# ayankele/dune-transformercvn

Measured on AMD Instinct MI355X. Metric: events/sec (fwd+bwd) at batch=32, 8 prongs/event; fraction of MFMA roofline, higher is better.
Workload: dtype bf16; 1 GPU; TransformerCVN DenseNet [3,6,12,6,3] g32, fwd+loss+bwd, batch 32/GPU, 8 prongs/event, 3x400x280 maps, 6-layer encoder, dropout 0.1; global_batch=32, parallelism=dp1, precision=bf16

## Files before the change

dune-transformercvn_amd/csrc/conv3x3_tile.hip:

```cpp
#include <cstdlib>
#include <type_traits>
#include "tile3x3.h"
#include "prof.h"

namespace tcvn {

using namespace t3;

namespace {


__device__ __forceinline__ int fdiv(int a, int d, float inv, int& rem) {
    int q = (int)((float)a * inv);
    rem = a - q * d;
    if (rem < 0) { --q; rem += d; }
    else if (rem >= d) { ++q; rem -= d; }
    return q;
}
__device__ __forceinline__ int pix_of(const PadGeom& q, int g, float invWp, float invHp) {
    if (g < 0 || g >= (int)q.gtot) return -1;
    int wp, hp;
    const int row = fdiv(g, q.Wp, invWp, wp);
    const int img = fdiv(row, q.Hp, invHp, hp);
    if (hp < 1 || hp > q.H || wp < 1 || wp > q.W) return -1;
// ... 294 lines not shown
    const int nrows4 = (q.rows() + 3) & ~3;
    int* tbl = reinterpret_cast<int*>(smem + ring * 256);
    float* xchg = reinterpret_cast<float*>(smem + ring * 256 + PAIR_TBL * 4);
    bf16* ctile = reinterpret_cast<bf16*>(xchg + 2 * 4 * 16 * 64);
    double* red = reinterpret_cast<double*>(ctile + 4 * 32 * 32);
    float* xtab = reinterpret_cast<float*>(red + 4 * 32 * 2);

    const int tid = threadIdx.x, lane = tid & 63, wave = tid >> 6;
    const bool roleB = wave >= 4;
    const bool xf = g.act_fused != 0;
    const int pw = wave & 3;
    const int r = lane & 31, h = lane >> 5;
    const float invWp = 1.0f / q.Wp, invHp = 1.0f / q.Hp;
    const bf16* __restrict__ YA = reinterpret_cast<const bf16*>(g.Aact);
    const char* __restrict__ zeros = reinterpret_cast<const char*>(g.zeros);
    bf16* __restrict__ Out = reinterpret_cast<bf16*>(g.Out);
    const int nb = gridDim.x, base = ntiles / nb, rem = ntiles % nb;
    const int t0 = blockIdx.x * base + min((int)blockIdx.x, rem), t1 = t0 + base + ((int)blockIdx.x < rem ? 1 : 0);
    const int g_org = t0 * TP - q.halo;
    const bool nok = r < g.N;
    const float bias = nok ? g.bias[r] : 0.f;
    const bool drop = g.drop_p > 0.f;
    const uint32_t dkey = drop_key(g.seed, g.stream_id);
    const bool vec_store = g.N == 32 && (g.n_off & 7) == 0 && (g.ldo & 7) == 0 && (reinterpret_cast<uintptr_t>(g.Out) & 15) == 0;
    auto wrap = [&](int x) { return x >= ring ? x - ring : x; };

    const bf16* __restrict__ Wf = reinterpret_cast<const bf16*>(g.Wfrag) + lane * 8;

    auto fill_rows = [&](int row0, int n, int t, int nt) {
        for (int i = t; i < n; i += nt) tbl[(row0 + i) & (PAIR_TBL - 1)] = pix_of(q, g_org + row0 + i, invWp, invHp);
    };
    auto dma_rows = [&](int row0, int slot0, int n, int w0, int nw) {
        const int rsub = lane >> 4, slot = lane & 15;
        for (int rg0 = w0; rg0 * 4 < n; rg0 += 4 * nw) {
            int m4[4];
#pragma unroll
            for (int j = 0; j < 4; ++j) m4[j] = tbl[(row0 + (rg0 + nw * j) * 4 + rsub) & (PAIR_TBL - 1)];
#pragma unroll
            for (int j = 0; j < 4; ++j) {
                const int rg = rg0 + nw * j;
                if (rg * 4 < n) {
                    const int ring_row = wrap(slot0 + rg * 4);
                    const int rr = ring_row + rsub;
                    const char* src = m4[j] >= 0 ? reinterpret_cast<const char*>(YA + (long)m4[j] * 128) + ((slot ^ (rr & 15)) << 4) : zeros + (slot << 4);
                    __builtin_amdgcn_global_load_lds((const __attribute__((address_space(1))) void*)src,
                                                     (__attribute__((address_space(3))) void*)(smem + ring_row * 256), 16, 0, 0);
// ... 20 lines not shown
            const Act8 tb = act8_load(xtab, cc);
#pragma unroll
            for (int j = 0; j < 4; ++j)
                if (m4[j] >= 0) *reinterpret_cast<u16x8*>(p[j]) = act8_apply(v[j], tb);
        }
    };
    if (t0 < t1) fill_rows(0, nrows4, tid, 512);
    if (t0 + 1 < t1) fill_rows(nrows4, TP, tid, 512);
    if (xf && g.lf.isum != nullptr) {
        if (tid < 128) {
            float tsc, tsh;
            lf_table(g.lf, tid, blockIdx.x == 0, tsc, tsh);
            xtab[tid] = tsc; xtab[128 + tid] = tsh; xtab[256 + tid] = g.sl[tid];
        }
    } else if (xf) act_tab_fill(xtab, g.sc, g.sh, g.sl, tid, 512);
    __syncthreads();
    if (t0 < t1) dma_rows(0, 0, nrows4, wave, 8);

#ifdef TCVN_DEBUG_KNOBS
    unsigned long long ph[16] = {0, 0, 0, 0, 0, 0, 0, 0, 0, 0, 0, 0, 0, 0, 0, 0};
#endif
    double s1 = 0, s2 = 0;
    f32x16 accp;
#pragma unroll
    for (int e = 0; e < 16; ++e) accp[e] = 0.f;
    int slot_tile = 0;
    int slot_new = wrap(nrows4);
    auto epilogue_impl = [&](auto dropc, auto vecc, int te, const f32x16& mine) {
        constexpr bool DROP = decltype(dropc)::value, VEC = decltype(vecc)::value;
        const float* xc = xchg + (((te - t0) & 1) * 4 + pw) * 16 * 64 + lane;
        float part[16];
#pragma unroll
        for (int e = 0; e < 16; ++e) part[e] = xc[e * 64];
        int mrow[16];
#pragma unroll
        for (int e = 0; e < 16; ++e) mrow[e] = tbl[((te - t0) * TP + q.halo + pw * 32 + (e & 3) + 8 * (e >> 2) + 4 * h) & (PAIR_TBL - 1)];
        float f1 = 0.f, f2 = 0.f;
        bf16* ct = ctile + pw * 32 * 32;
        uint32_t kword = 0;
#pragma unroll
        for (int e = 0; e < 16; ++e) {
            const int m = mrow[e];
            const bool ok = m >= 0 && nok;
            float v = mine[e] + part[e] + bias;
            if (DROP) {
                const int mm = m < 0 ? 0 : m;
                const float dsc = drop_pick(drop_bits32(dkey, mm, r, g.N), mm, g.drop_p);
                v *= dsc;
                const unsigned long long bal = __ballot(dsc != 0.f);
                kword = lane == 2 * e ? (uint32_t)bal : lane == 2 * e + 1 ? (uint32_t)(bal >> 32) : kword;
            }
            const bf16 o = ok ? f2bf(v) : (bf16)0;
            const float x = bf2f(o);
            f1 += x; f2 = fmaf(x, x, f2);
            if (VEC) ct[((e & 3) + 8 * (e >> 2) + 4 * h) * 32 + r] = o;
            else if (ok) Out[(long)m * g.ldo + g.n_off + r] = o;
        }
        s1 += (double)f1; s2 += (double)f2;
        if (DROP && g.keep_out != nullptr && lane < 32) {
            const int el = lane >> 1, pos = (el & 3) + 8 * (el >> 2) + 4 * (lane & 1);
            const int m = tbl[((te - t0) * TP + q.halo + pw * 32 + pos) & (PAIR_TBL - 1)];
            if (m >= 0) g.keep_out[m] = kword;
        }
        if (VEC) {
#pragma unroll
            for (int i = 0; i < 2; ++i) {
                const int c = lane + 64 * i, pos = c >> 2, chunk = c & 3;
                const int m = tbl[((te - t0) * TP + q.halo + pw * 32 + pos) & (PAIR_TBL - 1)];
                const u16x8 v8 = *reinterpret_cast<const u16x8*>(ct + pos * 32 + chunk * 8);
                if (m >= 0) *reinterpret_cast<u16x8*>(Out + (long)m * g.ldo + g.n_off + chunk * 8) = v8;
            }
        }
    };
    auto epilogue = [&](int te, const f32x16& mine) {
        if (drop) {
            if (vec_store) epilogue_impl(std::true_type{}, std::true_type{}, te, mine);
            else epilogue_impl(std::true_type{}, std::false_type{}, te, mine);
        } else {
            if (vec_store) epilogue_impl(std::false_type{}, std::true_type{}, te, mine);
            else epilogue_impl(std::false_type{}, std::false_type{}, te, mine);
        }
    };

    auto multiply = [&](auto& bwr, auto ntc, int tap_first, int slot_t, f32x16& acc) {
        constexpr int NT = decltype(ntc)::value, NG = NT * 2;
#pragma unroll
        for (int e = 0; e < 16; ++e) acc[e] = 0.f;
        const int lrow0 = slot_t + pw * 32 + r + q.halo;
        auto row_of = [&](int tp) {
            const int tap = tap_first + tp;
            int lr = lrow0 + (tap / 3 - 1) * q.Wp + (tap % 3 - 1);
            lr = lr >= ring ? lr - ring : lr;
            return lr >= ring ? lr - ring : lr;
        };
        bf16x8_t af[2][4];
        auto load_group = [&](int gI, bf16x8_t (&dst)[4]) {
            const int lr = row_of(gI >> 1), ks0 = (gI & 1) * 4;
#pragma unroll
            for (int i = 0; i < 4; ++i)
                dst[i] = *reinterpret_cast<const bf16x8_t*>(smem + lr * 256 + (((2 * (ks0 + i) + h) ^ (lr & 15)) << 4));
        };
        load_group(0, af[0]);
#pragma unroll
// ... 34 lines not shown
            if (t + 2 < t1) fill_rows(nrows4 + (t - t0 + 1) * TP, TP, tid, 256);
            PAIR_PH(4);
            slot_tile = wrap(slot_tile + TP);
            slot_new = wrap(slot_new + TP);
        }
    } else {
        bf16x8_t bw[32];
#pragma unroll
        for (int i = 0; i < 32; ++i) bw[i] = *reinterpret_cast<const bf16x8_t*>(Wf + (40 + i) * 512);
        __builtin_amdgcn_s_setprio(1);
        PAIR_T0();
        int slot_dma = 0;
        for (int t = t0; t < t1; ++t) {
            asm volatile("s_waitcnt vmcnt(0)" ::: "memory");
            if (xf) {
                if (t == t0) xform_rows(0, 0, nrows4, wave, 8);
                else xform_rows(nrows4 + (t - 1 - t0) * TP, slot_dma, TP, wave, 8);
            }
            PAIR_PH(8);
            __syncthreads();
            PAIR_PH(9);
            slot_dma = slot_new;
            if (xf && t + 1 < t1) dma_rows(nrows4 + (t - t0) * TP, slot_new, TP, wave, 8);
            PAIR_PH(10);
            if (t > t0) epilogue(t - 1, accp);
            PAIR_PH(11);
            multiply(bw, std::integral_constant<int, 4>{}, 5, slot_tile, accp);
            PAIR_PH(12);
            slot_tile = wrap(slot_tile + TP);
            slot_new = wrap(slot_new + TP);
        }
    }
#ifdef TCVN_DEBUG_KNOBS
    if (lane == 0 && (blockIdx.x & 15) == 0)
        for (int i = 0; i < 16; ++i)
            if (ph[i]) atomicAdd(&g_pair_ph[i], ph[i]);
#endif
    __syncthreads();
    if (roleB && t1 > t0) epilogue(t1 - 1, accp);
    if (g.part != nullptr || g.isum_out != nullptr) {
        double a = s1, b = s2;
        a += __shfl_xor(a, 32); b += __shfl_xor(b, 32);
        if (roleB && lane < 32) { red[(pw * 32 + lane) * 2] = a; red[(pw * 32 + lane) * 2 + 1] = b; }
        __syncthreads();
        if (tid < g.N) {
            double x = 0, y = 0;
#pragma unroll
            for (int w = 0; w < 4; ++w) { x += red[(w * 32 + tid) * 2]; y += red[(w * 32 + tid) * 2 + 1]; }
            if (g.isum_out != nullptr) lf_add(g.isum_out, g.isum_stride, tid, x, y);
            else {
                g.part[((long)blockIdx.x * g.N + tid) * 2] = x;
                g.part[((long)blockIdx.x * g.N + tid) * 2 + 1] = y;
            }
        }
    }
}
int fwd_pair_ring(const PadGeom& q) { return (int)((((q.rows() + 3) & ~3) + TP + 15) & ~15); }
size_t fwd_pair_smem(const PadGeom& q) { const size_t ring = fwd_pair_ring(q); return ring * 256 + PAIR_TBL * 4 + 2 * 4 * 16 * 64 * 4 + 4 * 32 * 32 * 2 + 4 * 32 * 16 + 3 * 128 * 4; }


size_t fwd_smem(const PadGeom& q) { const size_t r4 = (q.rows() + 3) & ~3; return 2 * r4 * 256 + 3 * r4 * 4 + 4 * 32 * 16; }

// ... 948 lines not shown
    return q.gtot < (1L << 24) && fwd_smem(q) <= 160 * 1024;
}
int conv3x3_tile_nblk(const ConvFwdArgs& a) {
    const PadGeom q(a.M / (a.H * a.W), a.H, a.W);
    return tile_grid(q.tiles());
}
static bool fwd_strip_forced() {
    static const bool on = TCVN_KNOB_SET("TCVN_FWD_STRIP");
    return on;
}
static bool fwd_pair_ok(const ConvFwdArgs& a, const PadGeom& q) {
    return fwd_pair_smem(q) <= 160 * 1024 && 4 * TP + q.halo + q.Wp + 1 < PAIR_TBL && (long)a.M * a.N < (1L << 32) && !fwd_strip_forced();
}
bool conv3x3_act_fusable(const ConvFwdArgs& a) {
    if (!conv3x3_tile_ok(a) || a.sc == nullptr || a.sh == nullptr || a.sl == nullptr) return false;
    static const bool off = TCVN_KNOB_SET("TCVN_NO_ACT_FUSE");
    const PadGeom q(a.M / (a.H * a.W), a.H, a.W);
    return !off && fwd_pair_ok(a, q) && wgrad_smem(q) <= 160 * 1024;
}
bool conv3x3_fwd_pair(const ConvFwdArgs& a) {
    if (!conv3x3_tile_ok(a)) return false;
    return fwd_pair_ok(a, PadGeom(a.M / (a.H * a.W), a.H, a.W));
}
bool conv3x3_fwd_writes_keep(const ConvFwdArgs& a) {
    if (a.keep_out == nullptr || a.drop_p <= 0.f || !conv3x3_tile_ok(a)) return false;
    return fwd_pair_ok(a, PadGeom(a.M / (a.H * a.W), a.H, a.W));
}
int conv3x3_fwd_tile(const ConvFwdArgs& a, hipStream_t st) {
    const int n_img = a.M / (a.H * a.W);
    const PadGeom q(n_img, a.H, a.W);
    const int ntiles = (int)q.tiles();
    const int nb = tile_grid(ntiles);
    const size_t smem = fwd_smem(q);
    static bool attr = false;
    if (!attr) {
        TCVN_CHECK(hipFuncSetAttribute(reinterpret_cast<const void*>(k_conv3x3_fwd_bf16), hipFuncAttributeMaxDynamicSharedMemorySize,
                                       160 * 1024));
        attr = true;
    }
    ProfScope ps("k_conv3x3_fwd_bf16", 2.0 * a.M * (double)a.N * a.K, (double)a.M * 2.0 * (a.C + a.N), st);
    if (fwd_pair_ok(a, q)) {
        static bool attr3 = false;
        if (!attr3) {
            TCVN_CHECK(hipFuncSetAttribute(reinterpret_cast<const void*>(k_conv3x3_fwd_pair_bf16), hipFuncAttributeMaxDynamicSharedMemorySize,
                                           160 * 1024));
            attr3 = true;
        }
        hipLaunchKernelGGL(k_conv3x3_fwd_pair_bf16, dim3(nb), dim3(512), fwd_pair_smem(q), st, a, n_img, ntiles, fwd_pair_ring(q));
        TCVN_LAUNCH_CHECK();
        return 0;
// ... 124 lines not shown
```

dune-transformercvn_amd/csrc/densenet.hip:

```cpp
#include <string>
#include <vector>
#include <cstring>

#include "../../include/tcvn_hip.h"
#include "tcvn_ops.h"
#include "tcvn_rows.h"
#include <cstdlib>
#include "densenet_plan.h"

using namespace tcvn;

namespace {
constexpr float kEps = 1e-5f, kMom = 0.1f;
}

int DenseNetPlan::add_slot(const std::string& name, long numel, int kind) {
    slots.push_back({name, numel, kind});
    return (int)slots.size() - 1;
}
BnSlots DenseNetPlan::add_bn(const std::string& p, int c) {
    BnSlots s;
    s.w = add_slot(p + ".weight", c, TCVN_SLOT_PARAM);
    s.b = add_slot(p + ".bias", c, TCVN_SLOT_PARAM);
    s.rm = add_slot(p + ".running_mean", c, TCVN_SLOT_BUFFER);
// ... 239 lines not shown
}

int DenseNetPlan::bind(void* const* d, void* const* g) {
    for (size_t i = 0; i < slots.size(); ++i) {
        data[i] = reinterpret_cast<float*>(d[i]);
        grad[i] = g ? reinterpret_cast<float*>(g[i]) : nullptr;
        if (slots[i].kind != TCVN_SLOT_COUNTER && data[i] == nullptr) {
            fprintf(stderr, "tcvn: slot %s unbound\n", slots[i].name.c_str());
            return -10;
        }
    }
    wk_cache = wk_list();
    fast3x3 = cfg.mode == MODE_BF16 && cfg.bn_size * cfg.growth == 128 && cfg.growth <= 32 && conv3x3_tile_enabled();
    bound = true;
    desc_ws = nullptr;
    undesc_ws = nullptr;
    return 0;
}

namespace {
struct Tab { float* sc; float* sh; };
}

int DenseNetPlan::upload_descs(char* ws, const Layout& L, hipStream_t st) {
    if (desc_ws == ws && desc_total == L.total) return 0;
    std::vector<PackDesc> pd;
    for (const auto& e : wk_cache) {
        PackDesc d;
        d.src = data[e.slot]; d.dst = ws + L.wk + e.off; d.N = e.N; d.Cin = e.Cin; d.taps = e.taps; d.Kp = e.Kp;
        d.transpose = e.transpose; d.frag = e.frag;
        pd.push_back(d);
    }
    std::vector<BnEvalDesc> bd;
    float* tabs = reinterpret_cast<float*>(ws + L.tabs);
    auto addbn = [&](const BnSlots& s) {
        BnEvalDesc d;
        d.gamma = data[s.w]; d.beta = data[s.b]; d.rm = data[s.rm]; d.rv = data[s.rv];
        d.sc = tabs + tab_off(s); d.sh = d.sc + round_up(s.C, 8); d.C = s.C;
        bd.push_back(d);
    };
    addbn(n0);
    for (const auto& bg : blocks) {
        for (const auto& ls : bg.layers) { addbn(ls.n1); addbn(ls.n2); }
        if (bg.has_trans) addbn(bg.tn);
    }
    addbn(nf);
    n_pack = (int)pd.size(); n_bneval = (int)bd.size();
    const size_t bytes = pd.size() * sizeof(PackDesc) + bd.size() * sizeof(BnEvalDesc);
    if (bytes > desc_cap) {
        if (d_desc) TCVN_CHECK(hipFree(d_desc));
        TCVN_CHECK(hipMalloc(&d_desc, bytes));
        desc_cap = bytes;
    }
    h_desc.resize(bytes);
    memcpy(h_desc.data(), pd.data(), pd.size() * sizeof(PackDesc));
    memcpy(h_desc.data() + pd.size() * sizeof(PackDesc), bd.data(), bd.size() * sizeof(BnEvalDesc));
    TCVN_CHECK(hipMemcpyAsync(d_desc, h_desc.data(), bytes, hipMemcpyHostToDevice, st));
    desc_ws = ws; desc_total = L.total;
    return 0;
}

int DenseNetPlan::forward(int n, const int32_t* coords, const float* values, long nnz, int log_pixels, float noise_std,
                          float* out, long out_ld, char* ws, long ws_bytes, int train, uint64_t seed, hipStream_t st) {
    if (!bound) return -11;
    if (n <= 0) return 0;
    Layout L;
    layout(n, train != 0, L);
    if (ws_bytes < L.total) { fprintf(stderr, "tcvn: densenet workspace too small (%ld < %ld)\n", ws_bytes, L.total); return -12; }
    int rc;
    if ((rc = upload_descs(ws, L, st))) return rc;
    const int mode = cfg.mode, g = cfg.growth, mid = cfg.bn_size * cfg.growth;
    float* tabs = reinterpret_cast<float*>(ws + L.tabs);
    auto tab = [&](const BnSlots& s) { Tab t; t.sc = tabs + tab_off(s); t.sh = t.sc + round_up(s.C, 8); return t; };
    double* part = reinterpret_cast<double*>(ws + L.part);
    const PackDesc* d_pack = reinterpret_cast<const PackDesc*>(d_desc);
    const BnEvalDesc* d_bn = reinterpret_cast<const BnEvalDesc*>(d_desc + n_pack * sizeof(PackDesc));

    if ((rc = pack_weights(d_pack, n_pack, mode, st))) return rc;
    if (!train && (rc = bn_eval_tables(d_bn, n_bneval, kEps, st))) return rc;

    auto link = [&](const BnSlots& s, const double* prt, int nblk, int part_ld, int c_new0, int n_new, double* bstat,
                    long count, const long long* isum = nullptr, long isum_stride = 0) -> int {
        if (!train) return 0;
        BnLinkArgs a{};
        a.isum = isum; a.isum_stride = isum_stride;
        a.part = prt; a.nblk = nblk; a.part_ld = part_ld; a.c_new0 = c_new0; a.n_new = n_new; a.bstat = bstat;
        a.count = count; a.C = s.C; a.gamma = data[s.w]; a.beta = data[s.b];
        a.running_mean = data[s.rm]; a.running_var = data[s.rv];
        Tab t = tab(s); a.sc = t.sc; a.sh = t.sh; a.train = 1; a.eps = kEps; a.momentum = kMom;
        return bn_link(a, st);
    };

    static const bool no_lf = TCVN_KNOB_SET("TCVN_NO_LF");
    const bool lf_on = train && !no_lf && mode == MODE_BF16 && L.isum_bytes > 0;
    TCVN_CHECK(hipMemsetAsync(ws + L.zeros, 0, 1024 + (lf_on ? L.isum_bytes : 0), st));
    auto lf_of = [&](const BnSlots& s, const long long* isum, long rep_stride, int c_new0, int n_new, double* bstat, long count) {
        LfLink k{};
        k.isum = isum; k.rep_stride = rep_stride; k.c_new0 = c_new0; k.n_new = n_new; k.bstat = bstat; k.inv_count = 1.0 / (double)count; k.count = count;
        k.gamma = data[s.w]; k.beta = data[s.b]; k.running_mean = data[s.rm]; k.running_var = data[s.rv];
        Tab t = tab(s); k.sc_out = t.sc; k.sh_out = t.sh; k.eps = kEps; k.momentum = kMom;
        return k;
    };
// ... 170 lines not shown
                if ((int)act_fused[bi].size() != bg.L) act_fused[bi].assign(bg.L, 0);
                act_fused[bi][l] = 0;
                if (mode == MODE_BF16) {
                    a.zeros = ws + L.zeros;
                    a.Aact = ws + L.Y[bi][l];
                    if (!fuse_ya && conv3x3_act_fusable(a)) { a.act_fused = 1; act_fused[bi][l] = 1; }
                    else {
                        if (!fuse_ya) {
                            ActArgs act{ws + L.Y[bi][l], mid, M, mid, t.sc, t.sh, data[ls.a2], ws + L.YA[bi][l], mid};
                            if ((rc = act_bf16(act, st))) return rc;
                        }
                        a.Aact = ws + L.YA[bi][l];
                    }
                }
                a.part = train ? part : nullptr;
                a.drop_p = train ? cfg.dropout : 0.f; a.seed = seed; a.stream_id = (uint32_t)(bi * 64 + l + 1);
                a.nblk = conv_fwd_nblk(a);
                if (lf2) {
                    if (!a.act_fused) { fprintf(stderr, "tcvn: link-free norm2 without the in-LDS activation\n"); return -17; }
                    a.lf = lf_of(ls.n2, reinterpret_cast<long long*>(ws + L.isumY[bi][l]), 2L * mid, 0, mid, reinterpret_cast<double*>(ws + L.bstatY[bi][l]), M);
                }
                const bool out_isum = lf_on && mode == MODE_BF16 && conv3x3_fwd_pair(a) && g <= 32;
                if (out_isum) { a.isum_out = isumD + 2 * ls.cin; a.isum_stride = 2L * bg.ld; }
                if (train && !L.KM[bi].empty()) {
                    a.keep_out = reinterpret_cast<uint32_t*>(ws + L.KM[bi][l]);
                    if (keep_valid.size() != blocks.size()) keep_valid.assign(blocks.size(), std::vector<char>());
                    if ((int)keep_valid[bi].size() != bg.L) keep_valid[bi].assign(bg.L, 0);
                    keep_valid[bi][l] = conv3x3_fwd_writes_keep(a) ? 1 : 0;
                }
                if ((rc = conv_fwd(a, st))) return rc;
                new_c0 = ls.cin; new_n = g; new_nblk = a.nblk; new_ld = g; new_isum = out_isum;
            }
        }
        if (bg.has_trans) {
            const BlockGeom& nb = blocks[bi + 1];
            if ((rc = link(bg.tn, part, new_nblk, new_ld, new_c0, new_n, bstatD, M, new_isum ? isumD + 2 * new_c0 : nullptr, 2L * bg.ld))) return rc;
            const WkEntry& e = wk_find(bg.tw, 0);
            Tab t = tab(bg.tn);
            const long Mn = (long)n * nb.H * nb.W;
            const bool fastt = L.XP[bi] >= 0 && mode == MODE_BF16;
            const bool mat32 = L.XP[bi] >= 0 && mode == MODE_F32;
            if (fastt || mat32) {
                ActPoolArgs ap{D, bg.ld, n, bg.H, bg.W, bg.Ctot, t.sc, t.sh, data[bg.ta], ws + L.XP[bi], bg.ldp};
                if ((rc = fastt ? act_pool_bf16(ap, st) : act_pool_f32(ap, st))) return rc;
            }
            if (fastt) {
                const WkEntry& ef = wk_find(bg.tw, 0, 1);
                GemmNtArgs ga{};
                ga.epi = EPI_FWD; ga.A = ws + L.XP[bi]; ga.lda = bg.ldp; ga.K = bg.ldp; ga.M = Mn; ga.N = bg.Ctot / 2;
                ga.Wfrag = ws + L.wk + ef.off; ga.Kp = ef.Kp; ga.zeros = ws + L.zeros; ga.bias = data[bg.tb];
                ga.Out = ws + L.D[bi + 1]; ga.ldo = nb.ld; ga.n_off = 0; ga.part = train ? part : nullptr; ga.nblk = gemm_nt_nblk(ga);
// ... 24 lines not shown
    if ((rc = linear_fwd(F, Cf, data[s_wl], nullptr, Z, cfg.out_dim, n, cfg.out_dim, Cf, st))) return rc;
    float* hs = reinterpret_cast<float*>(ws + L.head_stat);
    RowsBnArgs r{};
    r.X = Z; r.ldx = cfg.out_dim; r.R = n; r.C = cfg.out_dim; r.gamma = data[nl.w]; r.beta = data[nl.b]; r.slope = data[s_al];
    r.running_mean = data[nl.rm]; r.running_var = data[nl.rv]; r.Y = out; r.ldy = out_ld;
    r.save_mean = hs; r.save_rstd = hs + cfg.out_dim; r.train = train; r.eps = kEps; r.momentum = kMom;
    r.drop_p = train ? cfg.dropout : 0.f; r.seed = seed; r.stream_id = 0x4000u;
    if ((rc = rows_bn_fwd(r, st))) return rc;
    last_seed = seed; last_n = n; last_coords = coords; last_nnz = nnz;
    return 0;
}

int DenseNetPlan::tap(int n, const char* name, long* off, int* tn, int* th, int* tw, int* tc, int* tld, int* tes) const {
    Layout L;
    layout(n, false, L);
    std::string s(name);
    *tn = n; *tes = esz;
    if ((s == "img" || s == "conv0") && last_sparse_stem && n == last_n) return -1;
    if (s == "img") { *off = L.img; *th = cfg.H; *tw = cfg.W; *tc = cfg.in_ch; *tld = cfg.in_ch; return 0; }
    if (s == "conv0") { *off = L.c0; *th = Hc; *tw = Wc; *tc = cfg.init_ch; *tld = cfg.init_ch; return 0; }
    if (s == "condense") { *off = L.F; *th = 1; *tw = 1; *tc = Cf; *tld = Cf; *tes = 4; return 0; }
    if (s == "raw:wk") { *tn = *th = *tw = 1; *off = L.wk; *tc = *tld = (int)(wk_bytes() / esz); return 0; }
    if (s == "raw:tabs") { *tn = *th = *tw = 1; *off = L.tabs; *tc = *tld = (int)tab_floats(); *tes = 4; return 0; }
    if (s.rfind("raw:ystat", 0) == 0) {
        int b = 0, l = 0;
        if (sscanf(s.c_str(), "raw:ystat%d.%d", &b, &l) != 2) return -1;
        b -= 1;
        if (b < 0 || b >= (int)blocks.size() || l < 0 || l >= blocks[b].L) return -1;
        *tn = *th = *tw = 1; *off = L.bstatY[b][l]; *tc = *tld = 2 * cfg.bn_size * cfg.growth; *tes = 8; return 0;
    }
    if (s.rfind("raw:bstat", 0) == 0) {
        const int b = atoi(s.c_str() + 9) - 1;
        if (b < 0 || b >= (int)blocks.size()) return -1;
        *tn = *th = *tw = 1; *off = L.bstatD[b]; *tc = *tld = blocks[b].ld * 2; *tes = 8; return 0;
    }
    if (s.rfind("dense", 0) == 0) {
        const int b = atoi(s.c_str() + 5) - 1;
        if (b < 0 || b >= (int)blocks.size()) return -1;
        *off = L.D[b]; *th = blocks[b].H; *tw = blocks[b].W; *tc = blocks[b].Ctot; *tld = blocks[b].ld;
        return 0;
    }
    if (s.rfind("bottleneck", 0) == 0) {
        int b = 0, l = 0;
        if (sscanf(s.c_str(), "bottleneck%d.%d", &b, &l) != 2) return -1;
        b -= 1;
        if (b < 0 || b >= (int)blocks.size() || l < 0 || l >= blocks[b].L) return -1;
// ... 75 lines not shown
```

dune-transformercvn_amd/csrc/densenet_plan.h:

```cpp
#pragma once
#include <string>
#include <vector>

#include "../../include/tcvn_hip.h"
#include "tcvn_common.h"

namespace tcvn {

struct Bwd1x1Args;
struct Slot { std::string name; long numel; int kind; };
struct BnSlots { int w = -1, b = -1, rm = -1, rv = -1, nbt = -1, C = 0, id = -1; };
struct LayerSlots { BnSlots n1, n2; int a1, w1, b1, a2, w2, b2, cin; };
struct BlockGeom {
    int H, W, C0, L, Ctot, ld;
    int ldp;
    std::vector<LayerSlots> layers;
    bool has_trans = false;
    BnSlots tn; int ta = -1, tw = -1, tb = -1;
};
struct WkEntry { int slot, N, Cin, taps, transpose, rows, Kp, frag; long off; };

struct Layout {
    long img, c0, bstat0, part, tabs, F, Z, head_stat, wk, fwd_end, total;
    std::vector<long> D, bstatD;
// ... 10 lines not shown
    std::vector<std::vector<long>> XA;
    std::vector<long> XP;
    long du, du0, pq0, pqY, gwk, bpart, dF, dZ, zero_end;
    std::vector<long> G, pqD;
};

bool backward_overlap_enabled();
void set_backward_overlap(int on);

struct DenseNetPlan {
    tcvn_densenet_cfg cfg;
    int esz, Hc, Wc, Cf, n_bn = 0;
    std::vector<Slot> slots;
    std::vector<float*> data, grad;
    std::vector<BlockGeom> blocks;
    int s_w0, s_b0, s_a0, s_af, s_wl, s_al;
    BnSlots n0, nf, nl;
    std::vector<WkEntry> wk_cache;
    bool bound = false;
    bool fast1_ok(int cin) const;
    bool fastt_ok(int Ctot) const;
    bool fast3x3 = false;
    char* d_desc = nullptr; size_t desc_cap = 0; std::vector<char> h_desc;
    char* desc_ws = nullptr; long desc_total = 0; int n_pack = 0, n_bneval = 0;
    uint64_t last_seed = 0; int last_n = 0;
    const int32_t* last_coords = nullptr; long last_nnz = 0;
    const float* last_values = nullptr; int last_value_mode = 0; float last_noise = 0.f;
    std::vector<std::vector<char>> keep_valid;
    std::vector<std::vector<char>> act_fused;
    std::vector<std::vector<char>> xa_skipped;
    bool last_fused_ya = false;
    bool last_stem_act = false;
    bool last_sparse_stem = false;
    bool sparse_stem_possible() const;
    hipStream_t side_st = nullptr; hipEvent_t ev_fork_a = nullptr, ev_fork_b = nullptr, ev_done[2] = {nullptr, nullptr}, ev_drain = nullptr;
    int ensure_side();
    char* d_undesc = nullptr; std::vector<char> h_undesc; char* undesc_ws = nullptr; long undesc_total = 0; int n_unpack = 0;

    explicit DenseNetPlan(const tcvn_densenet_cfg& c);
    ~DenseNetPlan();
    int add_slot(const std::string& name, long numel, int kind);
    BnSlots add_bn(const std::string& p, int c);
    void layout(int n, bool bwd, Layout& L) const;
    void layout_bwd(int n, long start, long maxY, Layout& L) const;
    long tab_floats() const;
    long tab_off(const BnSlots& s) const;
    long wk_bytes() const;
    std::vector<WkEntry> wk_list() const;
    const WkEntry& wk_find(int slot, int transpose, int frag = 0) const;
    const void* wk_frag(const char* ws, const Layout& L, int slot, int transpose) const;
    int bind(void* const* d, void* const* g);
    int upload_descs(char* ws, const Layout& L, hipStream_t st);
    int forward(int n, const int32_t* coords, const float* values, long nnz, int log_pixels, float noise_std, float* out,
                long out_ld, char* ws, long ws_bytes, int train, uint64_t seed, hipStream_t st);
    int backward(int n, const float* d_out, long d_out_ld, char* ws, long ws_bytes, hipStream_t st, int bi_hi = -1, int bi_lo = 0);
    bool bwd1x1_fill(int bi, int l, long M, char* ws, const Layout& L, Bwd1x1Args& fa) const;
    bool bwd1x1_fusable(int bi, int l, long M, char* ws, const Layout& L) const;
    std::vector<int> unpack_first;
    int tap(int n, const char* name, long* off, int* tn, int* th, int* tw, int* tc, int* tld, int* tes) const;
};

}
```

dune-transformercvn_amd/csrc/elementwise.hip:

```cpp
#include "tcvn_ops.h"

namespace tcvn {

namespace {

__global__ __launch_bounds__(256) void k_bn_link(const BnLinkArgs a) {
    const int wave = threadIdx.x >> 6, lane = threadIdx.x & 63;
    const int c = blockIdx.x * 4 + wave;
    if (c >= a.C) return;
    const float gamma = a.gamma[c], beta = a.beta[c];
    const bool upd = a.train && a.running_mean != nullptr;
    const float rmean = upd || !a.train ? a.running_mean[c] : 0.f, rvar = upd || !a.train ? a.running_var[c] : 0.f;
    double mean, var;
    if (a.train) {
        if (c >= a.c_new0 && c < a.c_new0 + a.n_new && a.isum != nullptr) {
            long long sa, sb;
            lf_sums(a.isum, a.isum_stride, c - a.c_new0, sa, sb);
            mean = (double)sa * ((1.0 / (double)a.count) / LF_S1);
            var = (double)sb * ((1.0 / (double)a.count) / LF_S2) - mean * mean;
            if (var < 0) var = 0;
            if (lane == 0) { a.bstat[c * 2] = mean; a.bstat[c * 2 + 1] = var; }
        } else if (c >= a.c_new0 && c < a.c_new0 + a.n_new) {
            double s1 = 0, s2 = 0;
            for (int b = lane; b < a.nblk; b += 512) {
// ... 285 lines not shown
        const int r = (int)(q / kc8), k0 = (int)(q - (long)r * kc8) * 8;
        float v[8];
        int tap = k0 / inner, c = k0 - tap * inner;
#pragma unroll
        for (int j = 0; j < 8; ++j) {
            v[j] = 0.f;
            if (r < rows && k0 + j < klim)
                v[j] = d.transpose ? d.src[((long)c * d.Cin + r) * d.taps + tap] : d.src[((long)r * d.Cin + c) * d.taps + tap];
            if (++c == inner) { c = 0; ++tap; }
        }
        const long o = d.frag ? ((((long)(r >> 5) * (d.Kp >> 4) + (k0 >> 4)) * 64 + ((k0 >> 3) & 1) * 32 + (r & 31)) * 8) : (long)r * d.Kp + k0;
        if constexpr (sizeof(T) == 2) {
            u16x8 w;
#pragma unroll
            for (int j = 0; j < 8; ++j) w[j] = f2bf(v[j]);
            *reinterpret_cast<u16x8*>(dst + o) = w;
        } else {
            *reinterpret_cast<f32x4*>(dst + o) = f32x4{v[0], v[1], v[2], v[3]};
            *reinterpret_cast<f32x4*>(dst + o + 4) = f32x4{v[4], v[5], v[6], v[7]};
        }
    }
}


__global__ __launch_bounds__(256) void k_pool0_vec64(const Pool0Args a) {
    __shared__ double red[4][8][8][2];
    const bf16* X = reinterpret_cast<const bf16*>(a.X);
    bf16* O = reinterpret_cast<bf16*>(a.Out);
    const int tid = threadIdx.x, c8 = tid & 7;
    float sc[8], sh[8], sl[8];
#pragma unroll
    for (int j = 0; j < 8; ++j) { sc[j] = a.sc[c8 * 8 + j]; sh[j] = a.sh[c8 * 8 + j]; sl[j] = a.sl[c8 * 8 + j]; }
    double s1[8], s2[8];
#pragma unroll
    for (int j = 0; j < 8; ++j) { s1[j] = 0; s2[j] = 0; }
    const long npix = (long)a.n_img * a.Ho * a.Wo;
    for (long p = (long)blockIdx.x * 32 + (tid >> 3); p < npix; p += (long)gridDim.x * 32) {
        const int wo = (int)(p % a.Wo);
        const int ho = (int)((p / a.Wo) % a.Ho);
        const long img = p / ((long)a.Wo * a.Ho);
        const bf16* base = X + ((img * a.Hin + 2 * ho) * a.Win + 2 * wo) * 64 + c8 * 8;
        float acc[8] = {0, 0, 0, 0, 0, 0, 0, 0};
#pragma unroll
        for (int dy = 0; dy < 3; ++dy)
#pragma unroll
            for (int dx = 0; dx < 3; ++dx) {
// ... 94 lines not shown
    hipLaunchKernelGGL(k_act_pool_bf16, dim3((unsigned)(g < 4096 ? g : 4096)), dim3(256), 3 * cpr * 8 * sizeof(float), st, a);
    TCVN_LAUNCH_CHECK();
    return 0;
}

int act_pool_f32(const ActPoolArgs& a, hipStream_t st) {
    if ((a.ldx & 3) || (a.ldo & 3) || a.ldo < a.C || (reinterpret_cast<uintptr_t>(a.X) & 15) || (reinterpret_cast<uintptr_t>(a.Out) & 15)) return -2;
    const long total = (long)a.n_img * (a.Hin / 2) * (a.Win / 2) * (a.ldo >> 2);
    if (total <= 0) return 0;
    const long g = (total + 255) / 256;
    hipLaunchKernelGGL(k_act_pool_f32, dim3((unsigned)(g < 8192 ? g : 8192)), dim3(256), 0, st, a);
    TCVN_LAUNCH_CHECK();
    return 0;
}

int pack_weights(const PackDesc* d_descs, int n, int mode, hipStream_t st) {
    if (n <= 0) return 0;
    if (mode == MODE_F32) hipLaunchKernelGGL(k_pack<float>, dim3(256, n), dim3(256), 0, st, d_descs);
    else hipLaunchKernelGGL(k_pack<bf16>, dim3(256, n), dim3(256), 0, st, d_descs);
    TCVN_LAUNCH_CHECK();
    return 0;
}

}
```

dune-transformercvn_amd/csrc/tcvn_ops.h:

```cpp
#pragma once
#include "tcvn_common.h"
#include "bn_lf.h"

namespace tcvn {

enum AMode { A_1X1 = 0, A_1X1_POOL = 1, A_3X3 = 2, A_STEM = 3 };

struct ConvFwdArgs {
    int mode, amode;
    const void* A; long lda;
    int M, N, K, Kp;
    int C, H, W, Hin, Win;
    const float *sc, *sh, *sl;
    const void* Wk; const float* bias;
    void* Out; long ldo; int n_off;
    const void* Wfrag;
    const void* Aact;
    const void* zeros;
    double* part; int nblk;
    float drop_p; uint64_t seed; uint32_t stream_id;
    uint32_t* keep_out;
    int act_fused;
    LfLink lf;
    long long* isum_out; long isum_stride;
};
int conv_fwd(const ConvFwdArgs& a, hipStream_t st);
bool conv3x3_fwd_pair(const ConvFwdArgs& a);
bool conv3x3_fwd_writes_keep(const ConvFwdArgs& a);
bool conv3x3_act_fusable(const ConvFwdArgs& a);
int conv_fwd_grid(int M);
int conv_fwd_nblk(const ConvFwdArgs& a);
bool conv3x3_tile_ok(const ConvFwdArgs& a);
int conv3x3_tile_nblk(const ConvFwdArgs& a);
int conv3x3_fwd_tile(const ConvFwdArgs& a, hipStream_t st);
bool conv3x3_tile_enabled();

struct BnLinkArgs {
    const double* part; int nblk; int part_ld;
    int c_new0, n_new;
    double* bstat;
    long count;
    int C;
    const float *gamma, *beta;
    float *running_mean, *running_var;
    float *sc, *sh;
    int train; float eps, momentum;
    const long long* isum; long isum_stride;
};
int bn_link(const BnLinkArgs& a, hipStream_t st);

struct BnEvalDesc { const float *gamma, *beta, *rm, *rv; float *sc, *sh; int C; };
int bn_eval_tables(const BnEvalDesc* d_descs, int n, float eps, hipStream_t st);

struct ScatterArgs {
    int mode; const int* coords; const float* values; long nnz; int n_img;
    void* img; int H, W, Cpix; int log_pixels; float noise_std; uint64_t seed;
};
int scatter_pixels(const ScatterArgs& a, hipStream_t st);

struct Pool0Args {
    int mode; const void* X; int n_img, Hin, Win, C; const float *sc, *sh, *sl;
    void* Out; long ldo; int Ho, Wo; double* part; int nblk;
};
int pool0_fwd(const Pool0Args& a, hipStream_t st);
int pool0_grid(int n_img, int Ho, int Wo);

struct HeadPoolArgs { int mode; const void* X; long ldx; int n_img, HW, C; const float *sc, *sh, *sl; float* F; };
int head_pool_fwd(const HeadPoolArgs& a, hipStream_t st);

struct ActArgs { const void* X; long ldx; long M; int C; const float *sc, *sh, *sl; void* Out; long ldo; };
int act_bf16(const ActArgs& a, hipStream_t st);

struct PackDesc { const float* src; void* dst; int N, Cin, taps, Kp; int transpose; int frag; };
int pack_weights(const PackDesc* d_descs, int n, int mode, hipStream_t st);

struct EffSrc {
    const void* G; long ldg;
    const void* X; long ldx;
    int c_off, N;
    const float *P, *Q;
    float drop_p; uint64_t seed; uint32_t stream_id;
    const uint32_t* keep;
    const void* ey;
};

enum DMode { DG_1X1 = 0, DG_1X1_POOL = 1, DG_3X3 = 2 };
struct ConvDgradArgs {
    int mode, dmode;
    EffSrc e;
    int M, N, Kp;
    int H, W, Hin, Win;
    const void* Wt;
    const void* Xin; long ldxin;
    const float *sc, *sh, *sl;
    void* Gout; long ldgo; int accumulate;
    double* part; int nblk;
    const void* Wfrag;
// ... 187 lines not shown
```

Baseline: 1773 events/s.

## Precompute dropout keep masks in one batched kernel, read them in conv epilogue

Adds a batched k_keep_words kernel that produces the dropout keep bitmasks for every dense layer up front. The 3x3 tile conv epilogue then loads a prefetched keep word per row and applies the mask with readlane and inverse_ballot, instead of hashing random bits per element inside the MFMA-heavy kernel. This takes RNG work off the conv critical path at the cost of one extra launch and extra mask reads and writes. Computing masks inside the kernel is still available behind an env knob.

```diff
diff --git a/dune-transformercvn_amd/csrc/conv3x3_tile.hip b/dune-transformercvn_amd/csrc/conv3x3_tile.hip
--- a/dune-transformercvn_amd/csrc/conv3x3_tile.hip
+++ b/dune-transformercvn_amd/csrc/conv3x3_tile.hip
@@ -340,6 +340,8 @@
     const float bias = nok ? g.bias[r] : 0.f;
     const bool drop = g.drop_p > 0.f;
     const uint32_t dkey = drop_key(g.seed, g.stream_id);
+    const uint32_t* __restrict__ KM = g.keep_in;
+    const float dinv = 1.f / (1.f - g.drop_p);
     const bool vec_store = g.N == 32 && (g.n_off & 7) == 0 && (g.ldo & 7) == 0 && (reinterpret_cast<uintptr_t>(g.Out) & 15) == 0;
     auto wrap = [&](int x) { return x >= ring ? x - ring : x; };
 
@@ -406,12 +408,14 @@
 #endif
     double s1 = 0, s2 = 0;
     f32x16 accp;
+    uint32_t kw_next = 0;
 #pragma unroll
     for (int e = 0; e < 16; ++e) accp[e] = 0.f;
     int slot_tile = 0;
     int slot_new = wrap(nrows4);
-    auto epilogue_impl = [&](auto dropc, auto vecc, int te, const f32x16& mine) {
-        constexpr bool DROP = decltype(dropc)::value, VEC = decltype(vecc)::value;
+    auto epilogue_impl = [&](auto dropc, auto vecc, int te, const f32x16& mine, uint32_t kw) {
+        constexpr int DROP = decltype(dropc)::value;
+        constexpr bool VEC = decltype(vecc)::value;
         const float* xc = xchg + (((te - t0) & 1) * 4 + pw) * 16 * 64 + lane;
         float part[16];
 #pragma unroll
@@ -427,7 +431,11 @@
             const int m = mrow[e];
             const bool ok = m >= 0 && nok;
             float v = mine[e] + part[e] + bias;
-            if (DROP) {
+            if (DROP == 2) {
+                const int pos0 = (e & 3) + 8 * (e >> 2);
+                const uint32_t k0 = __builtin_amdgcn_readlane(kw, pos0), k1 = __builtin_amdgcn_readlane(kw, pos0 + 4);
+                v *= __builtin_amdgcn_inverse_ballot_w64(((unsigned long long)k1 << 32) | k0) ? dinv : 0.f;
+            } else if (DROP == 1) {
                 const int mm = m < 0 ? 0 : m;
                 const float dsc = drop_pick(drop_bits32(dkey, mm, r, g.N), mm, g.drop_p);
                 v *= dsc;
@@ -441,7 +449,7 @@
             else if (ok) Out[(long)m * g.ldo + g.n_off + r] = o;
         }
         s1 += (double)f1; s2 += (double)f2;
-        if (DROP && g.keep_out != nullptr && lane < 32) {
+        if (DROP == 1 && g.keep_out != nullptr && lane < 32) {
             const int el = lane >> 1, pos = (el & 3) + 8 * (el >> 2) + 4 * (lane & 1);
             const int m = tbl[((te - t0) * TP + q.halo + pw * 32 + pos) & (PAIR_TBL - 1)];
             if (m >= 0) g.keep_out[m] = kword;
@@ -456,13 +464,17 @@
             }
         }
     };
-    auto epilogue = [&](int te, const f32x16& mine) {
-        if (drop) {
-            if (vec_store) epilogue_impl(std::true_type{}, std::true_type{}, te, mine);
-            else epilogue_impl(std::true_type{}, std::false_type{}, te, mine);
+    auto epilogue = [&](int te, const f32x16& mine, uint32_t kw) {
+        using I0 = std::integral_constant<int, 0>; using I1 = std::integral_constant<int, 1>; using I2 = std::integral_constant<int, 2>;
+        if (drop && KM != nullptr) {
+            if (vec_store) epilogue_impl(I2{}, std::true_type{}, te, mine, kw);
+            else epilogue_impl(I2{}, std::false_type{}, te, mine, kw);
+        } else if (drop) {
+            if (vec_store) epilogue_impl(I1{}, std::true_type{}, te, mine, kw);
+            else epilogue_impl(I1{}, std::false_type{}, te, mine, kw);
         } else {
-            if (vec_store) epilogue_impl(std::false_type{}, std::true_type{}, te, mine);
-            else epilogue_impl(std::false_type{}, std::false_type{}, te, mine);
+            if (vec_store) epilogue_impl(I0{}, std::true_type{}, te, mine, kw);
+            else epilogue_impl(I0{}, std::false_type{}, te, mine, kw);
         }
     };
 
@@ -543,8 +555,13 @@
             PAIR_PH(9);
             slot_dma = slot_new;
             if (xf && t + 1 < t1) dma_rows(nrows4 + (t - t0) * TP, slot_new, TP, wave, 8);
+            const uint32_t kw = kw_next;
+            if (drop && KM != nullptr) {
+                const int m = lane < 32 ? tbl[((t - t0) * TP + q.halo + pw * 32 + lane) & (PAIR_TBL - 1)] : -1;
+                kw_next = m >= 0 ? KM[m] : 0u;
+            }
             PAIR_PH(10);
-            if (t > t0) epilogue(t - 1, accp);
+            if (t > t0) epilogue(t - 1, accp, kw);
             PAIR_PH(11);
             multiply(bw, std::integral_constant<int, 4>{}, 5, slot_tile, accp);
             PAIR_PH(12);
@@ -558,7 +575,7 @@
             if (ph[i]) atomicAdd(&g_pair_ph[i], ph[i]);
 #endif
     __syncthreads();
-    if (roleB && t1 > t0) epilogue(t1 - 1, accp);
+    if (roleB && t1 > t0) epilogue(t1 - 1, accp, kw_next);
     if (g.part != nullptr || g.isum_out != nullptr) {
         double a = s1, b = s2;
         a += __shfl_xor(a, 32); b += __shfl_xor(b, 32);
@@ -1553,10 +1570,6 @@
     if (!conv3x3_tile_ok(a)) return false;
     return fwd_pair_ok(a, PadGeom(a.M / (a.H * a.W), a.H, a.W));
 }
-bool conv3x3_fwd_writes_keep(const ConvFwdArgs& a) {
-    if (a.keep_out == nullptr || a.drop_p <= 0.f || !conv3x3_tile_ok(a)) return false;
-    return fwd_pair_ok(a, PadGeom(a.M / (a.H * a.W), a.H, a.W));
-}
 int conv3x3_fwd_tile(const ConvFwdArgs& a, hipStream_t st) {
     const int n_img = a.M / (a.H * a.W);
     const PadGeom q(n_img, a.H, a.W);
diff --git a/dune-transformercvn_amd/csrc/densenet.hip b/dune-transformercvn_amd/csrc/densenet.hip
--- a/dune-transformercvn_amd/csrc/densenet.hip
+++ b/dune-transformercvn_amd/csrc/densenet.hip
@@ -285,8 +285,8 @@
 struct Tab { float* sc; float* sh; };
 }
 
-int DenseNetPlan::upload_descs(char* ws, const Layout& L, hipStream_t st) {
-    if (desc_ws == ws && desc_total == L.total) return 0;
+int DenseNetPlan::upload_descs(int n_img, char* ws, const Layout& L, hipStream_t st) {
+    if (desc_ws == ws && desc_total == L.total && desc_n == n_img) return 0;
     std::vector<PackDesc> pd;
     for (const auto& e : wk_cache) {
         PackDesc d;
@@ -308,8 +308,22 @@
         if (bg.has_trans) addbn(bg.tn);
     }
     addbn(nf);
-    n_pack = (int)pd.size(); n_bneval = (int)bd.size();
-    const size_t bytes = pd.size() * sizeof(PackDesc) + bd.size() * sizeof(BnEvalDesc);
+    std::vector<KeepDesc> kd;
+    keep_max_M = 0;
+    keep_covered.assign(blocks.size(), std::vector<char>());
+    for (size_t bi = 0; bi < blocks.size(); ++bi) {
+        const BlockGeom& bg = blocks[bi];
+        const long M = (long)n_img * bg.H * bg.W;
+        keep_covered[bi].assign(bg.L, 0);
+        if (L.KM[bi].empty() || cfg.growth > 32 || M * cfg.growth >= (1L << 32)) continue;
+        for (int l = 0; l < bg.L; ++l) {
+            kd.push_back(KeepDesc{reinterpret_cast<uint32_t*>(ws + L.KM[bi][l]), M, (uint32_t)(bi * 64 + l + 1), cfg.growth});
+            keep_covered[bi][l] = 1;
+        }
+        keep_max_M = std::max(keep_max_M, M);
+    }
+    n_pack = (int)pd.size(); n_bneval = (int)bd.size(); n_keep = (int)kd.size();
+    const size_t bytes = pd.size() * sizeof(PackDesc) + bd.size() * sizeof(BnEvalDesc) + kd.size() * sizeof(KeepDesc);
     if (bytes > desc_cap) {
         if (d_desc) TCVN_CHECK(hipFree(d_desc));
         TCVN_CHECK(hipMalloc(&d_desc, bytes));
@@ -318,8 +332,9 @@
     h_desc.resize(bytes);
     memcpy(h_desc.data(), pd.data(), pd.size() * sizeof(PackDesc));
     memcpy(h_desc.data() + pd.size() * sizeof(PackDesc), bd.data(), bd.size() * sizeof(BnEvalDesc));
+    memcpy(h_desc.data() + pd.size() * sizeof(PackDesc) + bd.size() * sizeof(BnEvalDesc), kd.data(), kd.size() * sizeof(KeepDesc));
     TCVN_CHECK(hipMemcpyAsync(d_desc, h_desc.data(), bytes, hipMemcpyHostToDevice, st));
-    desc_ws = ws; desc_total = L.total;
+    desc_ws = ws; desc_total = L.total; desc_n = n_img;
     return 0;
 }
 
@@ -331,7 +346,7 @@
     layout(n, train != 0, L);
     if (ws_bytes < L.total) { fprintf(stderr, "tcvn: densenet workspace too small (%ld < %ld)\n", ws_bytes, L.total); return -12; }
     int rc;
-    if ((rc = upload_descs(ws, L, st))) return rc;
+    if ((rc = upload_descs(n, ws, L, st))) return rc;
     const int mode = cfg.mode, g = cfg.growth, mid = cfg.bn_size * cfg.growth;
     float* tabs = reinterpret_cast<float*>(ws + L.tabs);
     auto tab = [&](const BnSlots& s) { Tab t; t.sc = tabs + tab_off(s); t.sh = t.sc + round_up(s.C, 8); return t; };
@@ -341,6 +356,11 @@
 
     if ((rc = pack_weights(d_pack, n_pack, mode, st))) return rc;
     if (!train && (rc = bn_eval_tables(d_bn, n_bneval, kEps, st))) return rc;
+    const bool keep_on = train && cfg.dropout > 0.f && n_keep > 0;
+    if (keep_on && (rc = keep_words(reinterpret_cast<const KeepDesc*>(d_desc + n_pack * sizeof(PackDesc) + n_bneval * sizeof(BnEvalDesc)), n_keep,
+                                    keep_max_M, cfg.dropout, seed, st))) return rc;
+    keep_valid = keep_covered;
+    if (!keep_on) for (auto& kv : keep_valid) std::fill(kv.begin(), kv.end(), 0);
 
     auto link = [&](const BnSlots& s, const double* prt, int nblk, int part_ld, int c_new0, int n_new, double* bstat,
                     long count, const long long* isum = nullptr, long isum_stride = 0) -> int {
@@ -557,11 +577,10 @@
                 }
                 const bool out_isum = lf_on && mode == MODE_BF16 && conv3x3_fwd_pair(a) && g <= 32;
                 if (out_isum) { a.isum_out = isumD + 2 * ls.cin; a.isum_stride = 2L * bg.ld; }
-                if (train && !L.KM[bi].empty()) {
-                    a.keep_out = reinterpret_cast<uint32_t*>(ws + L.KM[bi][l]);
-                    if (keep_valid.size() != blocks.size()) keep_valid.assign(blocks.size(), std::vector<char>());
-                    if ((int)keep_valid[bi].size() != bg.L) keep_valid[bi].assign(bg.L, 0);
-                    keep_valid[bi][l] = conv3x3_fwd_writes_keep(a) ? 1 : 0;
+                if (keep_valid[bi][l]) {
+                    static const bool keep_in_kernel = TCVN_KNOB_SET("TCVN_KEEP_IN_KERNEL");
+                    if (keep_in_kernel) a.keep_out = reinterpret_cast<uint32_t*>(ws + L.KM[bi][l]);
+                    else a.keep_in = reinterpret_cast<const uint32_t*>(ws + L.KM[bi][l]);
                 }
                 if ((rc = conv_fwd(a, st))) return rc;
                 new_c0 = ls.cin; new_n = g; new_nblk = a.nblk; new_ld = g; new_isum = out_isum;
@@ -632,6 +651,14 @@
     if (s == "condense") { *off = L.F; *th = 1; *tw = 1; *tc = Cf; *tld = Cf; *tes = 4; return 0; }
     if (s == "raw:wk") { *tn = *th = *tw = 1; *off = L.wk; *tc = *tld = (int)(wk_bytes() / esz); return 0; }
     if (s == "raw:tabs") { *tn = *th = *tw = 1; *off = L.tabs; *tc = *tld = (int)tab_floats(); *tes = 4; return 0; }
+    if (s.rfind("raw:keep", 0) == 0) {
+        int b = 0, l = 0;
+        if (sscanf(s.c_str(), "raw:keep%d.%d", &b, &l) != 2) return -1;
+        b -= 1;
+        if (b < 0 || b >= (int)blocks.size() || l < 0 || l >= blocks[b].L || L.KM[b].empty()) return -1;
+        if (n != last_n || b >= (int)keep_valid.size() || l >= (int)keep_valid[b].size() || !keep_valid[b][l]) return -1;
+        *off = L.KM[b][l]; *th = blocks[b].H; *tw = blocks[b].W; *tc = *tld = 1; *tes = 4; return 0;
+    }
     if (s.rfind("raw:ystat", 0) == 0) {
         int b = 0, l = 0;
         if (sscanf(s.c_str(), "raw:ystat%d.%d", &b, &l) != 2) return -1;
diff --git a/dune-transformercvn_amd/csrc/densenet_plan.h b/dune-transformercvn_amd/csrc/densenet_plan.h
--- a/dune-transformercvn_amd/csrc/densenet_plan.h
+++ b/dune-transformercvn_amd/csrc/densenet_plan.h
@@ -56,7 +56,9 @@
     bool fastt_ok(int Ctot) const;
     bool fast3x3 = false;
     char* d_desc = nullptr; size_t desc_cap = 0; std::vector<char> h_desc;
-    char* desc_ws = nullptr; long desc_total = 0; int n_pack = 0, n_bneval = 0;
+    char* desc_ws = nullptr; long desc_total = 0; int desc_n = 0, n_pack = 0, n_bneval = 0, n_keep = 0;
+    long keep_max_M = 0;
+    std::vector<std::vector<char>> keep_covered;
     uint64_t last_seed = 0; int last_n = 0;
     const int32_t* last_coords = nullptr; long last_nnz = 0;
     const float* last_values = nullptr; int last_value_mode = 0; float last_noise = 0.f;
@@ -84,7 +86,7 @@
     const WkEntry& wk_find(int slot, int transpose, int frag = 0) const;
     const void* wk_frag(const char* ws, const Layout& L, int slot, int transpose) const;
     int bind(void* const* d, void* const* g);
-    int upload_descs(char* ws, const Layout& L, hipStream_t st);
+    int upload_descs(int n_img, char* ws, const Layout& L, hipStream_t st);
     int forward(int n, const int32_t* coords, const float* values, long nnz, int log_pixels, float noise_std, float* out,
                 long out_ld, char* ws, long ws_bytes, int train, uint64_t seed, hipStream_t st);
     int backward(int n, const float* d_out, long d_out_ld, char* ws, long ws_bytes, hipStream_t st, int bi_hi = -1, int bi_lo = 0);
diff --git a/dune-transformercvn_amd/csrc/elementwise.hip b/dune-transformercvn_amd/csrc/elementwise.hip
--- a/dune-transformercvn_amd/csrc/elementwise.hip
+++ b/dune-transformercvn_amd/csrc/elementwise.hip
@@ -331,6 +331,25 @@
     }
 }
 
+__global__ __launch_bounds__(256) void k_keep_words(const KeepDesc* descs, float p, uint64_t seed) {
+    const KeepDesc d = descs[blockIdx.y];
+    const int lane = threadIdx.x & 63, wave = threadIdx.x >> 6;
+    const uint32_t key = drop_key(seed, d.stream_id);
+    const uint32_t thr = (uint32_t)(p * 65536.0f + 0.5f);
+    const long nchunk = (d.M + 63) >> 6;
+    for (long c = (long)blockIdx.x * 4 + wave; c < nchunk; c += (long)gridDim.x * 4) {
+        const int m0 = (int)(c << 6);
+        uint32_t w = 0;
+#pragma unroll
+        for (int j = 0; j < 16; ++j) {
+            const uint32_t bits = drop_bits32(key, m0 + 4 * j + 2 * (lane >> 5), lane & 31, d.N);
+            const unsigned long long lo = __ballot((bits & 0xffffu) >= thr), hi = __ballot((bits >> 16) >= thr);
+            const uint32_t w01 = (lane & 1) ? (uint32_t)hi : (uint32_t)lo, w23 = (lane & 1) ? (uint32_t)(hi >> 32) : (uint32_t)(lo >> 32);
+            if ((lane >> 2) == j) w = (lane & 2) ? w23 : w01;
+        }
+        if (m0 + lane < d.M) d.km[m0 + lane] = w;
+    }
+}
 
 __global__ __launch_bounds__(256) void k_pool0_vec64(const Pool0Args a) {
     __shared__ double red[4][8][8][2];
@@ -471,4 +490,12 @@
     return 0;
 }
 
-}
+int keep_words(const KeepDesc* d_descs, int n, long max_M, float p, uint64_t seed, hipStream_t st) {
+    if (n <= 0 || max_M <= 0) return 0;
+    const long g = (max_M + 255) / 256;
+    hipLaunchKernelGGL(k_keep_words, dim3((unsigned)(g < 1024 ? g : 1024), n), dim3(256), 0, st, d_descs, p, seed);
+    TCVN_LAUNCH_CHECK();
+    return 0;
+}
+
+}
diff --git a/dune-transformercvn_amd/csrc/tcvn_ops.h b/dune-transformercvn_amd/csrc/tcvn_ops.h
--- a/dune-transformercvn_amd/csrc/tcvn_ops.h
+++ b/dune-transformercvn_amd/csrc/tcvn_ops.h
@@ -19,6 +19,7 @@
     const void* zeros;
     double* part; int nblk;
     float drop_p; uint64_t seed; uint32_t stream_id;
+    const uint32_t* keep_in;
     uint32_t* keep_out;
     int act_fused;
     LfLink lf;
@@ -26,7 +27,6 @@
 };
 int conv_fwd(const ConvFwdArgs& a, hipStream_t st);
 bool conv3x3_fwd_pair(const ConvFwdArgs& a);
-bool conv3x3_fwd_writes_keep(const ConvFwdArgs& a);
 bool conv3x3_act_fusable(const ConvFwdArgs& a);
 int conv_fwd_grid(int M);
 int conv_fwd_nblk(const ConvFwdArgs& a);
@@ -73,6 +73,9 @@
 
 struct PackDesc { const float* src; void* dst; int N, Cin, taps, Kp; int transpose; int frag; };
 int pack_weights(const PackDesc* d_descs, int n, int mode, hipStream_t st);
+
+struct KeepDesc { uint32_t* km; long M; uint32_t stream_id; int N; };
+int keep_words(const KeepDesc* d_descs, int n, long max_M, float p, uint64_t seed, hipStream_t st);
 
 struct EffSrc {
     const void* G; long ldg;
```

Result: no change. 1771 events/s (-0.1%).
